# taqu/cpprcoder

Measured on AMD Instinct MI355X. Metric: MB/s encode+decode per GPU on 64 KiB blocks; ratio vs CPU ref, higher is better.
Workload: dtype u32

## Files before the change

### cpprcoder_amd/csrc/rcx_quad.hpp

```cpp
#pragma once

template <int CTRL>
__device__ __forceinline__ u32 rcx_dpp(u32 x)
{
    return (u32)__builtin_amdgcn_update_dpp(0, (int)x, CTRL, 0xF, 0xF, true);
}
__device__ __forceinline__ u32 rcx_oct_sum(u32 x)
{
    x += rcx_dpp<0xB1>(x);
    x += rcx_dpp<0x4E>(x);
    x += rcx_dpp<0x141>(x);
    return x;
}
__device__ __forceinline__ u32 rcx_oct_excl_scan(u32 x, u32 m1, u32 m2, u32 m4)
{
    u32 tot = x, pre = 0, o;
    o = rcx_dpp<0xB1>(tot);
    pre += o & m1;
    tot += o;
    o = rcx_dpp<0x4E>(tot);
    pre += o & m2;
    tot += o;
    o = rcx_dpp<0x141>(tot);
    pre += o & m4;
    return pre;
}

#define RCX_QUAD_BLOCKS 16
#define RCX_QUAD_GROUP_BYTES 4352
#define RCX_QUAD_RING_BYTES 144
#define RCX_QUAD_LDS_BYTES (4 * RCX_QUAD_GROUP_BYTES + RCX_QUAD_BLOCKS * RCX_QUAD_RING_BYTES)

typedef u32 RcxV4 __attribute__((ext_vector_type(4)));
typedef __attribute__((address_space(3))) RcxV4 RcxLdsV4;
typedef __attribute__((address_space(3))) u32 RcxLdsU32;
typedef RcxV4 RcxDivQv;
typedef RcxLdsV4 RcxLdsDivQ;

#define RCX_QUAD_DIVQ_DW 32

__device__ __forceinline__ u32 rcx_quad_sum(u32 x)
{
    x += rcx_dpp<0xB1>(x);
    x += rcx_dpp<0x4E>(x);
    return x;
}
__device__ __forceinline__ u32 rcx_umin(u32 a, u32 b) { return a < b ? a : b; }
__device__ __forceinline__ u32 rcx_umax(u32 a, u32 b) { return a > b ? a : b; }
__device__ __forceinline__ u32 rcx_quad_min(u32 x)
{
    x = rcx_umin(x, rcx_dpp<0xB1>(x));
    x = rcx_umin(x, rcx_dpp<0x4E>(x));
    return x;
}
__device__ __forceinline__ u32 rcx_quad_max(u32 x)
{
    x = rcx_umax(x, rcx_dpp<0xB1>(x));
    x = rcx_umax(x, rcx_dpp<0x4E>(x));
    return x;
}
__device__ __forceinline__ u32 rcx_quad_or(u32 x)
{
    x |= rcx_dpp<0xB1>(x);
    x |= rcx_dpp<0x4E>(x);
    return x;
}
__device__ __forceinline__ u32 rcx_quad_excl_scan(u32 x, u32 m1, u32 m2)
{
    u32 o = rcx_dpp<0xB1>(x);
    u32 pre = o & m1;
    const u32 tot = x + o;
    o = rcx_dpp<0x4E>(tot);
    pre += o & m2;
    return pre;
}

#if !defined(RCX_TOPUP_PIECES)
#define RCX_TOPUP_PIECES 1
#endif
struct QuadInput {
    u32 low, range;
    u32 bp8;
    u32 w0, w1;
    u32 n4;
    u32* ring;
    U4* skipped;
    u32 wr;
    u32 nfit;
    U4 pendA, pendB;
    const u8* origin;
    u32 last_off;
    u32 body8;

    __device__ __forceinline__ U4 load16(u32 off) const
    {
        return *reinterpret_cast<const U4*>(origin + (off < last_off ? off : last_off));
    }
    __device__ __forceinline__ void ring_put(const U4& piece, bool really)
    {
        const u32 slot = wr % RCX_RING_DW;
        *(really ? reinterpret_cast<U4*>(ring + slot) : skipped) = piece;
        ring[really && slot == 0 ? RCX_RING_DW : RCX_RING_DW + 1] = piece.x;
        wr += really ? 4u : 0u;
    }
    __device__ __forceinline__ void fetch_pair()
    {
        const u32* at = ring + ((bp8 >> 5) % RCX_RING_DW);
        w0 = at[0];
        w1 = at[1];
    }
    __device__ __forceinline__ u32 begin(const u8* s, const u8* stream_end, u32* block_ring, U4* scratch16)
    {
        skipped = scratch16;
        const u32 declared = (u32)s[0] | ((u32)s[1] << 8) | ((u32)s[2] << 16) | ((u32)s[3] << 24);
        low = ((u32)s[4] << 24) | ((u32)s[5] << 16) | ((u32)s[6] << 8) | (u32)s[7];
        range = 0x00FFFFFFu;
        ring = block_ring;
        const u8* body = s + 8;
        origin = body - ((uintptr_t)body & 15);
        last_off = (u32)(stream_end - 1 - origin) & ~15u;
        wr = 0;
        for (u32 r = 0; r < 6; ++r) ring_put(load16(16 * r), true);
        nfit = 0;
        pendA.x = pendA.y = pendA.z = pendA.w = 0;
        pendB = pendA;
        body8 = 8u * (u32)(body - origin);
        bp8 = body8;
        fetch_pair();
        n4 = rcx_bswap(rcx_funnel_shr(w1, w0, bp8));
        return declared;
    }
    __device__ __forceinline__ void idle(const u8* anywhere, u32* block_ring, U4* scratch16)
    {
        skipped = scratch16;
        low = 0;
        range = 0x01000000u;
        ring = block_ring;
        origin = anywhere - ((uintptr_t)anywhere & 15);
        last_off = 0;
        wr = 24;
        nfit = 0;
        pendA.x = pendA.y = pendA.z = pendA.w = 0;
        pendB = pendA;
        body8 = bp8 = 0;
        w0 = w1 = n4 = 0;
    }
    __device__ __forceinline__ void topup()
    {
        ring_put(pendA, nfit >= 1);
#if RCX_TOPUP_PIECES > 1
        ring_put(pendB, nfit >= 2);
#endif
        const u32 rd = bp8 >> 5;
        if (rcx_any(wr - rd < 14u)) {
            asm volatile("" ::: "memory");
            while (__any(wr - rd <= 20u)) ring_put(load16(4 * wr), wr - rd <= 20u);
        }
        const u32 room = (rd + RCX_RING_DW - wr) >> 2;
        nfit = room < (u32)RCX_TOPUP_PIECES ? room : (u32)RCX_TOPUP_PIECES;
        pendA = load16(4 * wr);
#if RCX_TOPUP_PIECES > 1
        pendB = load16(4 * wr + 16);
#endif
    }
    __device__ __forceinline__ u64 taken() const { return 8 + (u64)((bp8 - body8) >> 3); }
};

struct QuadSeat {
    u32 lane, wave;
    u32 quad, j;
    bool in_use;
    u64 blk;
    u8* lds;
    u8* mine;
    U4* leaves;
    U4* parked;
    u32* ring;
};
#define RCX_QUAD_SEAT(SEAT, WAVES, QUADS_USED, LDS_ALL, GEOM, NBLOCKS, N, BLOCK)                                       \
    QuadSeat SEAT;                                                                                                     \
    SEAT.lane = threadIdx.x & 63u;                                                                                     \
    SEAT.wave = __builtin_amdgcn_readfirstlane(threadIdx.x >> 6);                                                      \
    SEAT.lds = (LDS_ALL) + SEAT.wave * RCX_QUAD_LDS_BYTES;                                                             \
    SEAT.j = SEAT.lane & 3u, SEAT.quad = SEAT.lane >> 2;                                                               \
    SEAT.in_use = SEAT.quad < (QUADS_USED);                                                                            \
    SEAT.blk = ((u64)blockIdx.x * (WAVES) + SEAT.wave) * (QUADS_USED) + (SEAT.quad & ((QUADS_USED)-1u));               \
    RCX_ENTRY(GEOM, SEAT.blk, NBLOCKS, N, BLOCK);                                                                      \
    {                                                                                                                  \
                     \
        const u32 group = 2u * (SEAT.quad >> 3) + ((0x96u >> (SEAT.quad & 7u)) & 1u), quarter = (SEAT.quad & 7u) >> 1; \
        SEAT.mine = SEAT.lds + group * RCX_QUAD_GROUP_BYTES + quarter * 64;                                            \
        SEAT.leaves = reinterpret_cast<U4*>(SEAT.mine) + SEAT.j;                                                       \
        SEAT.parked = reinterpret_cast<U4*>(SEAT.mine + 16 * 256);                                                     \
        SEAT.ring = reinterpret_cast<u32*>(SEAT.lds + 4 * RCX_QUAD_GROUP_BYTES + SEAT.quad * RCX_QUAD_RING_BYTES);     \
    }

#define RCX_QUAD_FAIL(SEAT, GEOM, STATUS)                                                                              \
    {                                                                                                                  \
        if (SEAT.j == 0 && SEAT.in_use) rcx_flag(STATUS, RCX_ST_CORRUPT, rcx_id(GEOM, SEAT.blk));                      \
        live = false;                                                                                                  \
        len = 0;                                                                                                       \
    }
#define RCX_QUAD_MARK_REDO(SEAT, REDO, NBLOCKS, MARKED)                                                                \
    if (leader) (REDO)[SEAT.blk] = (MARKED) ? 1u : 0u;                                                                 \
    else if (SEAT.j == 0 && SEAT.in_use && SEAT.blk < (NBLOCKS)) (REDO)[SEAT.blk] = 0

#define RCX_QUAD_PARKED_FLUSH(I0, PARKED, LAST, ANY_ALIGN)                                                             \
    const u32 g = ((I0) >> 4) & 3u;                                                                                    \
    if (g == 0 && (I0) != 0 && leader) {                                                                               \
        u8* o4 = out + ((I0)-64);                                                                                      \
        const U4 p0 = (PARKED)[0], p1 = (PARKED)[1], p2 = (PARKED)[2];                                                 \
        rcx_store16<ANY_ALIGN>(o4, p0);                                                                                \
        rcx_store16<ANY_ALIGN>(o4 + 16, p1);                                                                           \
        rcx_store16<ANY_ALIGN>(o4 + 32, p2);                                                                           \
        rcx_store16<ANY_ALIGN>(o4 + 48, LAST);                                                                         \
    }
#define RCX_QUAD_PARKED_PUT(O, PARKED, LAST)                                                                           \
    if (g == 3) LAST = O;                                                                                              \
    else (PARKED)[g] = O
#define RCX_QUAD_PARKED_END(END, PARKED, LAST, ANY_ALIGN)                                                              \
    if (leader && (END) != 0) {                                                                                        \
        const u32 groups = (((END)-1) >> 4 & 3u) + 1;                                                                  \
        u8* o4 = out + (((END)-1) & ~63u);                                                                             \
        rcx_store16<ANY_ALIGN>(o4, (PARKED)[0]);                                                                       \
        if (groups > 1) rcx_store16<ANY_ALIGN>(o4 + 16, (PARKED)[1]);                                                  \
        if (groups > 2) rcx_store16<ANY_ALIGN>(o4 + 32, (PARKED)[2]);                                                  \
        if (groups > 3) rcx_store16<ANY_ALIGN>(o4 + 48, LAST);                                                         \
    }

#define RCX_QP1 "quad_perm:[1,0,3,2] row_mask:0xf bank_mask:0xf bound_ctrl:1\n\t"
#define RCX_QP2 "quad_perm:[2,3,0,1] row_mask:0xf bank_mask:0xf bound_ctrl:1\n\t"

#define RCX_QUAD_ROUND2_CUM(V, Q1, Q2, Q3, Q4)                                                                         \
    u32 lo_, rg_, nb_, hi_, y1_, y2_, y3_, y4_;                                                                       \
    asm volatile("v_sub_co_u32_e64 %[y1], %[c1], %[v], %[q1]\n\t"                                                     \
                 "v_sub_co_u32_e64 %[y2], %[c2], %[v], %[q2]\n\t"                                                     \
                 "v_sub_co_u32_e64 %[y3], %[c3], %[v], %[q3]\n\t"                                                     \
                 "v_sub_co_u32_e64 %[y4], %[c4], %[v], %[q4]\n\t"                                                     \
                 "v_subb_co_u32_e64 %[nb], %[c1], 4, 0, %[c1]\n\t"                                                    \
                 "v_min3_u32 %[lo], %[y1], %[y2], %[y3]\n\t"                                                          \
                 "v_subb_co_u32_e64 %[nb], %[c2], %[nb], 0, %[c2]\n\t"                                                \
                 "v_max3_u32 %[hi], %[y1], %[y2], %[y3]\n\t"                                                          \
                 "v_subb_co_u32_e64 %[nb], %[c3], %[nb], 0, %[c3]\n\t"                                                \
                 "v_min3_u32 %[lo], %[lo], %[y4], %[rem]\n\t"                                                         \
                 "v_subb_co_u32_e64 %[nb], %[c4], %[nb], 0, %[c4]\n\t"                                                \
                 "v_max_u32 %[hi], %[hi], %[y4]\n\t"                                                                  \
                 "v_min_u32_dpp %[lo], %[lo], %[lo] " RCX_QP1                                                         \
                 "v_add_u32_dpp %[nb], %[nb], %[nb] " RCX_QP1                                                         \
                 "v_max_u32_dpp %[hi], %[hi], %[hi] " RCX_QP1                                                         \
                 "v_min_u32_dpp %[lo], %[lo], %[lo] " RCX_QP2                                                         \
                 "v_add_u32_dpp %[nb], %[nb], %[nb] " RCX_QP2                                                         \
                 "v_max_u32_dpp %[hi], %[hi], %[hi] " RCX_QP2                                                         \
                 "v_sub_u32 %[rg], %[lo], %[hi]"                                                                      \
                 : [lo] "=&v"(lo_), [rg] "=&v"(rg_), [nb] "=&v"(nb_), [hi] "=&v"(hi_), [y1] "=&v"(y1_),               \
                   [y2] "=&v"(y2_), [y3] "=&v"(y3_), [y4] "=&v"(y4_), [c1] "=&s"(c1_), [c2] "=&s"(c2_),               \
                   [c3] "=&s"(c3_), [c4] "=&s"(c4_)                                                                   \
                 : [v] "v"(V), [q1] "v"(Q1), [q2] "v"(Q2), [q3] "v"(Q3), [q4] "v"(Q4),                                \
                   [rem] "v"(rem_));;

#define RCX_QUAD_16_SYMBOLS(SYMBOL, FINISH)                                                                            \
    SYMBOL(0, w0_, 0) SYMBOL(1, w0_, 0) SYMBOL(1, w0_, 8) SYMBOL(1, w0_, 16)                                           \
    SYMBOL(1, w0_, 24) SYMBOL(1, w1_, 0) SYMBOL(1, w1_, 8) SYMBOL(1, w1_, 16)                                          \
    SYMBOL(1, w1_, 24) SYMBOL(1, w2_, 0) SYMBOL(1, w2_, 8) SYMBOL(1, w2_, 16)                                          \
    SYMBOL(1, w2_, 24) SYMBOL(1, w3_, 0) SYMBOL(1, w3_, 8) SYMBOL(1, w3_, 16)                                          \
    FINISH(w3_, 24)

#define RCX_QUAD_TAIL(FROM, EACH, SYMBOL, FINISH, GATHER)                                                              \
    for (u32 i = (FROM); i < maxlen; ++i) {                                                                            \
        if ((i & 15u) == 0) in.topup();                                                                                \
        EACH                                                                                                           \
        if (i < len) {                                                                \
            u32 sym = 0;                                                                                               \
            SYMBOL(0, sym, 0);                                                                                         \
            FINISH(sym, 0);                                                                                            \
            sym = GATHER(sym);                                                                                         \
            if (leader) out[i] = (u8)sym;                                                                              \
        }                                                                                                              \
    }

#define RCX_QUAD_DEC_WAVES 4
template <int WAVES, class G = RcxBlocks>
__global__ __launch_bounds__(64 * WAVES) void rcx_dec_quad_k(const u8* __restrict__ comp, u64 comp_size, const u64* __restrict__ offsets,
                                                             u64 nblocks, u32 block, u64 n, u8* __restrict__ dst,
                                                             const u32* __restrict__ divq, u32* status,
                                                             u32* __restrict__ redo, u32 quads_used, const G g = G())
{
    __shared__ __attribute__((aligned(256))) u8 lds_all[WAVES * RCX_QUAD_LDS_BYTES];
    RCX_QUAD_SEAT(seat, WAVES, quads_used, lds_all, g, nblocks, n, block);

    {
        U4 v;
        v.x = v.y = v.z = v.w = ~0u;
#pragma unroll
        for (u32 q = 0; q < 17; ++q) seat.leaves[q * 16] = v;
    }
    u32 nU1 = 0u - (64u * seat.j + 16), nU2 = nU1 - 16, nU3 = nU1 - 32, nU4 = nU1 - 48;
    const u32 T0 = 4u * seat.j;
    const u32 m1 = (seat.j & 1u) ? ~0u : 0u, m2 = (seat.j & 2u) ? ~0u : 0u;

    QuadInput in;
    u64 stream_len = 0;
    if (live) {
        RCX_STREAM(g, seat.blk, offsets);
        if (!RCX_STREAM_OK(comp_size, 9)) {
            RCX_QUAD_FAIL(seat, g, status)
        } else {
            const u32 declared = in.begin(comp + s0, comp + s1, seat.ring, seat.parked + 3);
            if (declared != len) {
                RCX_QUAD_FAIL(seat, g, status)
            }
        }
    }
    if (!live) in.idle(comp, seat.ring, seat.parked + 3);

    const u32 maxlen = rcx_wave_max(len);
    u8* out = dst + at;
    u32 fast_end;
    {
        u32 mine = live ? (len & ~15u) : 0xFFFFFFF0u;
        if (!G::items && live && (reinterpret_cast<uintptr_t>(out) & 15u) != 0) mine = 0;
#pragma unroll
        for (int o = 32; o > 0; o >>= 1) {
            const u32 other = (u32)__shfl_xor((int)mine, o, 64);
            mine = mine < other ? mine : other;
        }
        fast_end = mine == 0xFFFFFFF0u ? 0u : mine;
    }
    const bool leader = live && seat.in_use && seat.j == 0;

    const u32 T0p3x4 = 4u * (T0 + 3);
    const u32 leaves_lds = (u32)reinterpret_cast<uintptr_t>(seat.leaves);
    const u32 ring_lds = (u32)reinterpret_cast<uintptr_t>(seat.ring);
#if defined(RCX_STAMP_DEC)
#define RCX_QUAD_STAMP(i) if (stamp_now_) stamp_t_[stamp_at_ + (i)] = __builtin_amdgcn_s_memtime();
#define RCX_QUAD_NO_STAMP                                                 \
    const bool stamp_now_ = false;                                                                         \
    const int stamp_at_ = 0;                                                                               \
    unsigned long long stamp_t_[4];
#else
#define RCX_QUAD_STAMP(i)
#define RCX_QUAD_NO_STAMP
#endif
    u32 p_hs_ = 0, p_sb4_ = 0, p_la_ = leaves_lds, p_own_ = 0;
#define RCX_QD_R_LO "v116"
#define RCX_QD_R_PAIR "{v[116:117]}"
    u64 R_ = 0;
#define RCX_QD_D "v[118:119]"
#define RCX_QD_D_L "v118"
#define RCX_QD_D_H "v119"
#define RCX_QD_YA "v[120:121]"
#define RCX_QD_YA_L "v120"
#define RCX_QD_YA_H "v121"
#define RCX_QD_YB "v[122:123]"
#define RCX_QD_YB_L "v122"
#define RCX_QD_YB_H "v123"
#define RCX_QD_YC "v[124:125]"
#define RCX_QD_YC_L "v124"
#define RCX_QD_YC_H "v125"
#define RCX_QD_YE "v[126:127]"
#define RCX_QD_YE_L "v126"
#define RCX_QD_YE_H "v127"
#define RCX_QD_PAIRS_CLOBBERED "v118", "v119", "v120", "v121", "v122", "v123", "v124", "v125", "v126", "v127"
#define RCX_QD_PREV_A_0 "s_nop 1\n\t"
#define RCX_QD_PREV_A_1 "v_lshl_add_u32 %[psym4], %[phs], 2, %[psb4]\n\t"                                           \
                        "v_bfi_b32 %[pad], 12, %[psym4], %[pla]\n\t"
#define RCX_QD_PREV_S_FIRST "v_and_b32 %[pword], %[psym4], %[pown]\n\t"                                             \
                            "v_lshrrev_b32 %[pword], 2, %[pword]\n\t"
#define RCX_QD_PREV_S_NEXT "v_and_b32 %[pye], %[psym4], %[pown]\n\t"                                                \
                           "v_lshl_or_b32 %[pword], %[pye], %[psh], %[pword]\n\t"
#define RCX_QP3 "quad_perm:[3,2,1,0] row_mask:0xf bank_mask:0xf bound_ctrl:1\n\t"
 \
#define RCX_QD_REM(PREV, PSHIFT, ...)                                                                      \
        asm volatile("v_min3_u32 %[rm], %[x1], %[x2], %[x3]\n\t"                                           \
                     "v_min3_u32 %[rm], %[rm], %[x4], %[low]\n\t"                                          \
                     "v_add_u32 %[u1], %[u1], %[h1]\n\t"                                                   \
                     "v_add_u32 %[u2], %[u2], %[h2]\n\t"                                                   \
                     "v_min_u32_dpp %[rm], %[rm], %[rm] " RCX_QP1                                          \
                     "v_add_u32 %[u3], %[u3], %[h3]\n\t"                                                   \
                     "v_add_u32 %[u4], %[u4], %[h4]\n\t"                                                   \
                     "v_min_u32_dpp " RCX_QD_R_LO ", %[rm], %[rm] " RCX_QP2  \
                     PREV                                                                                  \
                     : [u1] "+v"(nU1), [u2] "+v"(nU2), [u3] "+v"(nU3), [u4] "+v"(nU4), [rm] "=&v"(rem_),    \
                       [R] "+" RCX_QD_R_PAIR(R_) __VA_ARGS__                                                \
                     : [low] "v"(in.low), [x1] "v"(x1_), [x2] "v"(x2_),                                    \
                       [x3] "v"(x3_), [x4] "v"(x4_), [h1] "v"(h1_), [h2] "v"(h2_), [h3] "v"(h3_), [h4] "v"(h4_), \
                       [pown] "v"(p_own_), [psym4] "v"(psym4_), [psh] "n"((PSHIFT) > 2 ? (PSHIFT)-2 : 0))
#define RCX_QUAD_DEC_SYMBOL(MUL, INC, SH, HP, PWORD, PSHIFT)                                               \
    {                                                                                                      \
            \
        const u32 k8_ = rcx_clz(in.range) & 0x18u;                                                         \
        in.low = (u32)((((u64)in.low << 32) | in.n4) << k8_ >> 32);                                        \
                  \
        const u32 t_ = __umulhi((in.range << k8_) + (INC), (MUL)) >> (SH);                                 \
                                  \
        const u64 lowp_ = in.low;                                                                          \
        u32 node_, rem_, ro_, la_, pad_, pye_, psym4_;                                                     \
        u64 X1_, X2_, X3_, X4_, cz_, cy_;                                                                  \
        asm volatile("v_mad_i64_i32 %[X1], %[cz], %[n1], %[t], %[lp]\n\t"                                  \
                     "v_mad_i64_i32 %[X2], %[cz], %[n2], %[t], %[lp]\n\t"                                  \
                     "v_mad_i64_i32 %[X3], %[cz], %[n3], %[t], %[lp]\n\t"                                  \
                     "v_mad_i64_i32 %[X4], %[cz], %[n4], %[t], %[lp]"                                      \
                     : [X1] "=&v"(X1_), [X2] "=&v"(X2_), [X3] "=&v"(X3_), [X4] "=&v"(X4_), [cz] "=&s"(cz_)  \
                     : [n1] "v"(nU1), [n2] "v"(nU2), [n3] "v"(nU3), [n4] "v"(nU4), [t] "v"(t_), [lp] "v"(lowp_)); \
                                    \
        __builtin_amdgcn_sched_barrier(0);                                                                 \
        in.bp8 += k8_;                                                                                     \
        __builtin_amdgcn_sched_barrier(0);                                                                 \
        const u32 x1_ = (u32)X1_, x2_ = (u32)X2_, x3_ = (u32)X3_, x4_ = (u32)X4_;                          \
        const u32 h1_ = (u32)(X1_ >> 32), h2_ = (u32)(X2_ >> 32), h3_ = (u32)(X3_ >> 32), h4_ = (u32)(X4_ >> 32); \
        asm volatile("v_add3_u32 %[nd], %[h1], %[h2], %[h3]\n\t"                                           \
                     "v_add3_u32 %[nd], %[nd], %[h4], 4\n\t"  \
                     RCX_QD_PREV_A_##HP                                                                    \
                     : [nd] "=&v"(node_), [pad] "=&v"(pad_), [psym4] "=&v"(psym4_)                          \
                     : [h1] "v"(h1_), [h2] "v"(h2_), [h3] "v"(h3_), [h4] "v"(h4_),                         \
                       [phs] "v"(p_hs_), [psb4] "v"(p_sb4_), [pla] "v"(p_la_));                            \
        if (HP) (void)__hip_atomic_fetch_add(reinterpret_cast<RcxLdsU32*>(pad_), p_own_, __ATOMIC_RELAXED, __HIP_MEMORY_SCOPE_WAVEFRONT);  \
        asm volatile("v_add_u32_dpp %[nd], %[nd], %[nd] " RCX_QP1                                          \
                     "v_bfe_u32 %[ro], %[bp], 5, 5\n\t"                 \
                     "v_lshl_add_u32 %[ro], %[ro], 2, %[rb]"  \
                     : [nd] "+v"(node_), [ro] "=&v"(ro_)                                                    \
                     : [bp] "v"(in.bp8), [rb] "v"(ring_lds));                                              \
        {                                                                                                  \
            const RcxLdsU32* at_ = reinterpret_cast<const RcxLdsU32*>(ro_);  \
            in.w0 = at_[0];                                                                                \
            in.w1 = at_[1];                                                                                \
        }                                                                                                  \
        __builtin_amdgcn_sched_barrier(0);                                                                 \
        asm volatile("v_add_u32_dpp %[nd], %[nd], %[nd] " RCX_QP2                                          \
                     "v_lshl_add_u32 %[la], %[nd], 8, %[lvb]"  \
                     : [nd] "+v"(node_), [la] "=&v"(la_)                                                    \
                     : [lvb] "v"(leaves_lds));                                                             \
                                                              \
        RCX_QUAD_STAMP(0);                                                                                 \
        const RcxV4 l_ = *reinterpret_cast<const RcxLdsV4*>(la_);                                          \
        __builtin_amdgcn_sched_barrier(0);                                                                 \
        if (!(HP)) RCX_QD_REM("", 0);                                                                      \
        else if ((PSHIFT) == 0) RCX_QD_REM(RCX_QD_PREV_S_FIRST, 0, , [pword] "=&v"(PWORD));                \
        else RCX_QD_REM(RCX_QD_PREV_S_NEXT, PSHIFT, , [pye] "=&v"(pye_), [pword] "+v"(PWORD));             \
         \
         \
        u32 qe_, pre_, o2_, o3_;                                                                           \
        u32 lo_, rg_, hi_;                                                                                 \
        asm volatile("v_add3_u32 %[qe], %[lx], %[ly], %[lz]\n\t"                                           \
                     "v_add_u32 %[qe], %[qe], %[lw]\n\t"                                                   \
                     "v_alignbit_b32 %[n4], %[w1], %[w0], %[bp]\n\t"  \
                     "v_perm_b32 %[n4], %[n4], %[n4], %[swap]\n\t"  \
                     "v_and_b32_dpp %[pre], %[qe], %[m1] " RCX_QP1  \
                     "v_and_b32_dpp %[o2], %[qe], %[m2] " RCX_QP2                                          \
                     "v_and_b32_dpp %[o3], %[qe], %[m2] " RCX_QP3                                          \
                     "v_add3_u32 %[qe], %[pre], %[o2], %[o3]\n\t"                                         \
                     "v_mad_i64_i32 " RCX_QD_D ", %[cy], %[qe], %[t], %[R]\n\t"                             \
                     "v_mad_i64_i32 " RCX_QD_YA ", %[cy], %[lx], %[t], " RCX_QD_D "\n\t"                    \
                     "v_mad_i64_i32 " RCX_QD_YB ", %[cy], %[ly], %[t], " RCX_QD_YA "\n\t"                   \
                     "v_mad_i64_i32 " RCX_QD_YC ", %[cy], %[lz], %[t], " RCX_QD_YB "\n\t"                   \
                     "v_mad_i64_i32 " RCX_QD_YE ", %[cy], %[lw], %[t], " RCX_QD_YC "\n\t"                   \
                     "v_min3_u32 %[lo], " RCX_QD_D_L ", " RCX_QD_YA_L ", " RCX_QD_YB_L "\n\t"              \
                     "v_max3_u32 %[hi], " RCX_QD_YA_L ", " RCX_QD_YB_L ", " RCX_QD_YC_L "\n\t"             \
                     "v_min_u32 %[lo], %[lo], " RCX_QD_YC_L "\n\t"                                         \
                     "v_max_u32 %[hi], %[hi], " RCX_QD_YE_L "\n\t"                                         \
                     "v_add3_u32 %[hs], " RCX_QD_YA_H ", " RCX_QD_YB_H ", " RCX_QD_YC_H "\n\t"  \
                     "v_min_u32_dpp %[lo], %[lo], %[lo] " RCX_QP1                                          \
                     "v_max_u32_dpp %[hi], %[hi], %[hi] " RCX_QP1                                          \
                     "v_bfi_b32 %[own], " RCX_QD_D_H ", 0, " RCX_QD_YE_H "\n\t"  \
                     "v_min_u32_dpp %[lo], %[lo], %[lo] " RCX_QP2                                          \
                     "v_max_u32_dpp %[hi], %[hi], %[hi] " RCX_QP2                                          \
                     "v_sub_u32 %[rg], %[lo], %[hi]"                                                       \
                     : [n4] "=&v"(in.n4), [qe] "=&v"(qe_), [pre] "=&v"(pre_), [o2] "=&v"(o2_), [o3] "=&v"(o3_), \
                       [lo] "=&v"(lo_), [rg] "=&v"(rg_), [hs] "=&v"(p_hs_), [own] "=&v"(p_own_), [hi] "=&v"(hi_), \
                       [cy] "=&s"(cy_)                                                                      \
                     : [lx] "v"(l_.x), [ly] "v"(l_.y), [lz] "v"(l_.z), [lw] "v"(l_.w), [t] "v"(t_),        \
                       [R] "v"(R_), [m1] "v"(m1), [m2] "v"(m2),                                            \
                       [w0] "v"(in.w0), [w1] "v"(in.w1), [bp] "v"(in.bp8), [swap] "s"(0x00010203u)         \
                     : RCX_QD_PAIRS_CLOBBERED);                                                            \
                                  \
        __builtin_amdgcn_sched_barrier(0);                                                                 \
        p_sb4_ = (node_ << 6) + T0p3x4;                                                                    \
        __builtin_amdgcn_sched_barrier(0);                                                                 \
        asm volatile("" : : "v"(p_sb4_), "v"(qe_), "v"(pre_), "v"(o2_), "v"(o3_), "v"(hi_) : RCX_QD_PAIRS_CLOBBERED); \
        RCX_QUAD_STAMP(1);                                                                                 \
        in.low = lo_;                                                                            \
        in.range = rg_;                                                                          \
        p_la_ = la_;                                                                                       \
    }
#define RCX_QD_FINISH(BYTE, SHIFT, ...)                                                                    \
        asm volatile(RCX_QD_PREV_A_1                                                                       \
                     BYTE                                                                                  \
                     : [pad] "=&v"(pad_), [psym4] "=&v"(psym4_) __VA_ARGS__                                 \
                     : [pown] "v"(p_own_), [phs] "v"(p_hs_), [psb4] "v"(p_sb4_), [pla] "v"(p_la_),         \
                       [psh] "n"((SHIFT) > 2 ? (SHIFT)-2 : 0))
#define RCX_QUAD_DEC_FINISH(WORD, SHIFT)                                                                    \
    {                                                                                                      \
        u32 pad_, pye_, psym4_;                                                                            \
        if ((SHIFT) == 0) RCX_QD_FINISH(RCX_QD_PREV_S_FIRST, 0, , [pword] "=&v"(WORD));                    \
        else RCX_QD_FINISH(RCX_QD_PREV_S_NEXT, SHIFT, , [pye] "=&v"(pye_), [pword] "+v"(WORD));            \
        (void)__hip_atomic_fetch_add(reinterpret_cast<RcxLdsU32*>(pad_), p_own_, __ATOMIC_RELAXED, __HIP_MEMORY_SCOPE_WAVEFRONT);  \
    }

#if defined(RCX_QUAD_DIV_SMEM)
    const u32* dq_ = divq;
#else
    u32 vz_;
    asm volatile("v_mov_b32 %0, 0" : "=v"(vz_));
    const u32* dq_ = divq + vz_;
#endif
#define RCX_QUAD_DIVQ_LOAD(G, Q)                                                                             \
    {                                                                                                      \
        __builtin_amdgcn_sched_barrier(0);                                                                 \
        dm##Q = reinterpret_cast<const U4*>(dq_ + (G) * RCX_QUAD_DIVQ_DW)[Q];                              \
        di##Q = reinterpret_cast<const U4*>(dq_ + (G) * RCX_QUAD_DIVQ_DW + 16)[Q];                         \
    }
#define RCX_QUAD_U4_AT(V, C) ((C) == 0 ? (V).x : (C) == 1 ? (V).y : (C) == 2 ? (V).z : (V).w)
    {
        U4 o_last;
        o_last.x = o_last.y = o_last.z = o_last.w = 0;
#if defined(RCX_STAMP_DEC)
        unsigned long long stamp_sum_[4] = {0, 0, 0, 0};
#endif
        U4 dm0, dm1, dm2, dm3, di0, di1, di2, di3;
        RCX_QUAD_DIVQ_LOAD(0u, 0) RCX_QUAD_DIVQ_LOAD(0u, 1) RCX_QUAD_DIVQ_LOAD(0u, 2) RCX_QUAD_DIVQ_LOAD(0u, 3)
        asm volatile("" ::"v"(dm0.x), "v"(di0.x), "v"(dm1.x), "v"(di1.x), "v"(dm2.x), "v"(di2.x), "v"(dm3.x), "v"(di3.x));
#if defined(RCX_STAMP_DEC)
#define RCX_QUAD_STEP(S, Q, HP, PW)                                                                           \
    {                                                                                                        \
        const bool stamp_now_ = (S) == 8 || (S) == 9;                                                        \
        const int stamp_at_ = (S) == 8 ? 0 : 2;                                                              \
        RCX_QUAD_DEC_SYMBOL(RCX_QUAD_U4_AT(dm##Q, (S) & 3), RCX_QUAD_U4_AT(di##Q, (S) & 3), sh_, HP, PW,     \
                            (8 * (((S) + 3) & 3)));                                                          \
    }
#else
#define RCX_QUAD_STEP(S, Q, HP, PW)                                                                           \
    RCX_QUAD_DEC_SYMBOL(RCX_QUAD_U4_AT(dm##Q, (S) & 3), RCX_QUAD_U4_AT(di##Q, (S) & 3), sh_, HP, PW, (8 * (((S) + 3) & 3)));
#endif
#define RCX_QUAD_GROUP(GN, O)                                                                                 \
    {                                                                                                        \
        u32 w0_ = 0, w1_ = 0, w2_ = 0, w3_ = 0;                                                              \
        RCX_QUAD_STEP(0, 0, 0, w0_) RCX_QUAD_STEP(1, 0, 1, w0_) RCX_QUAD_STEP(2, 0, 1, w0_) RCX_QUAD_STEP(3, 0, 1, w0_) \
        RCX_QUAD_DIVQ_LOAD(GN, 0)                                                                            \
        RCX_QUAD_STEP(4, 1, 1, w0_) RCX_QUAD_STEP(5, 1, 1, w1_) RCX_QUAD_STEP(6, 1, 1, w1_) RCX_QUAD_STEP(7, 1, 1, w1_) \
        RCX_QUAD_DIVQ_LOAD(GN, 1)                                                                            \
        RCX_QUAD_STEP(8, 2, 1, w1_) RCX_QUAD_STEP(9, 2, 1, w2_) RCX_QUAD_STEP(10, 2, 1, w2_) RCX_QUAD_STEP(11, 2, 1, w2_) \
        RCX_QUAD_DIVQ_LOAD(GN, 2)                                                                            \
        RCX_QUAD_STEP(12, 3, 1, w2_) RCX_QUAD_STEP(13, 3, 1, w3_) RCX_QUAD_STEP(14, 3, 1, w3_) RCX_QUAD_STEP(15, 3, 1, w3_) \
        RCX_QUAD_DIVQ_LOAD(GN, 3)                                                                            \
        RCX_QUAD_DEC_FINISH(w3_, 24)                                                                         \
        (O).x = rcx_quad_or(w0_);                                                                            \
        (O).y = rcx_quad_or(w1_);                                                                            \
        (O).z = rcx_quad_or(w2_);                                                                            \
        (O).w = rcx_quad_or(w3_);                                                                            \
    }
        u32 i0 = 0;
#if !defined(RCX_STAMP_DEC)
        {
            U4 o_p0 = o_last, o_p1 = o_last, o_p2 = o_last;
            for (; i0 + 64 <= fast_end; i0 += 64) {
                in.topup();
                if (i0 != 0 && leader) {
                    u8* o4 = out + (i0 - 64);
                    rcx_store16<G::items>(o4, o_p0);
                    rcx_store16<G::items>(o4 + 16, o_p1);
                    rcx_store16<G::items>(o4 + 32, o_p2);
                    rcx_store16<G::items>(o4 + 48, o_last);
                }
                const u32 sh_ = 31u - (u32)__builtin_clz(256u + i0);
                const u32 gn_ = (i0 >> 4) + 1u;
                RCX_QUAD_GROUP(gn_, o_p0)
                in.topup();
                RCX_QUAD_GROUP(gn_ + 1u, o_p1)
                in.topup();
                RCX_QUAD_GROUP(gn_ + 2u, o_p2)
                in.topup();
                RCX_QUAD_GROUP(gn_ + 3u, o_last)
            }
            if (i0 != 0) seat.parked[0] = o_p0, seat.parked[1] = o_p1, seat.parked[2] = o_p2;
        }
#endif
        for (; i0 < fast_end; i0 += 16) {
            in.topup();
            RCX_QUAD_PARKED_FLUSH(i0, seat.parked, o_last, G::items)
            const u32 sh_ = 31u - (u32)__builtin_clz(256u + i0);
            const u32 gn_ = (i0 >> 4) + 1u;
#if defined(RCX_STAMP_DEC)
            unsigned long long stamp_t_[4] = {0, 0, 0, 0};
#endif
            U4 o;
            RCX_QUAD_GROUP(gn_, o)
#if defined(RCX_STAMP_DEC)
            stamp_sum_[0] += stamp_t_[1] - stamp_t_[0];
            stamp_sum_[1] += stamp_t_[2] - stamp_t_[1];
            stamp_sum_[2] += stamp_t_[3] - stamp_t_[2];
            stamp_sum_[3] += 1;
#endif
            RCX_QUAD_PARKED_PUT(o, seat.parked, o_last);
        }
#undef RCX_QUAD_GROUP
#undef RCX_QUAD_STEP
#if defined(RCX_STAMP_DEC)
        if (blockIdx.x == 7 && threadIdx.x == 0)
            for (int i_ = 0; i_ < 4; ++i_) rcx_dec_stamp_out[i_] = stamp_sum_[i_];
#endif
        RCX_QUAD_PARKED_END(fast_end, seat.parked, o_last, G::items)
    }
    {
        u32 mul_n_, inc_n_;
#define RCX_QUAD_DIVQ_ENTRY(I)                                                                              \
    {                                                                                                      \
        const u32* e_ = divq + ((I) >> 4) * RCX_QUAD_DIVQ_DW + ((I) & 15u);                                 \
        mul_n_ = e_[0];                                                                                    \
        inc_n_ = e_[16];                                                                                   \
    }
        RCX_QUAD_DIVQ_ENTRY(fast_end);
#define RCX_QUAD_TAIL_EACH                                                                                  \
    const u32 mul_ = mul_n_, inc_ = inc_n_, sh_ = 31u - (u32)__builtin_clz(256u + i);                      \
    RCX_QUAD_DIVQ_ENTRY(i + 1u);                                                                           \
    RCX_QUAD_NO_STAMP
#define RCX_QUAD_TAIL_SYMBOL(HP, WORD, SHIFT) RCX_QUAD_DEC_SYMBOL(mul_, inc_, sh_, HP, WORD, SHIFT)
        RCX_QUAD_TAIL(fast_end, RCX_QUAD_TAIL_EACH, RCX_QUAD_TAIL_SYMBOL, RCX_QUAD_DEC_FINISH, rcx_quad_or)
#undef RCX_QUAD_TAIL_EACH
#undef RCX_QUAD_TAIL_SYMBOL
    }
#undef RCX_QUAD_DEC_SYMBOL
#undef RCX_QUAD_DEC_FINISH
#undef RCX_QD_PREV_A_0
#undef RCX_QD_PREV_A_1
#undef RCX_QD_PREV_S_FIRST
#undef RCX_QD_PREV_S_NEXT
#undef RCX_QD_REM
#undef RCX_QD_FINISH
#undef RCX_QD_R_LO
#undef RCX_QD_R_PAIR
#undef RCX_QD_D
#undef RCX_QD_D_L
#undef RCX_QD_D_H
#undef RCX_QD_YA
#undef RCX_QD_YA_L
#undef RCX_QD_YA_H
#undef RCX_QD_YB
#undef RCX_QD_YB_L
#undef RCX_QD_YB_H
#undef RCX_QD_YC
#undef RCX_QD_YC_L
#undef RCX_QD_YC_H
#undef RCX_QD_YE
#undef RCX_QD_YE_L
#undef RCX_QD_YE_H
#undef RCX_QD_PAIRS_CLOBBERED
#undef RCX_QP3
#undef RCX_QUAD_DIVQ_LOAD
#undef RCX_QUAD_DIVQ_ENTRY
#undef RCX_QUAD_U4_AT
    const bool marked = live && rcx_quad_or(seat.j == 3 && 0u - nU4 != 256u + len ? 1u : 0u) != 0;
    if (leader && !marked && in.taken() > stream_len) rcx_flag(status, RCX_ST_CORRUPT, rcx_id(g, seat.blk));
    RCX_QUAD_MARK_REDO(seat, redo, nblocks, marked);
}
```

Before: 84250.

## Overlap quad-group merge with next group's first symbol decode; scalarize loop bounds

Result: no change. 84150 (-0.1%).

```diff
diff --git a/cpprcoder_amd/csrc/rcx_quad.hpp b/cpprcoder_amd/csrc/rcx_quad.hpp
--- a/cpprcoder_amd/csrc/rcx_quad.hpp
+++ b/cpprcoder_amd/csrc/rcx_quad.hpp
@@ -152,7 +152,7 @@
         ring_put(pendB, nfit >= 2);
 #endif
         const u32 rd = bp8 >> 5;
-        if (rcx_any(wr - rd < 14u)) {
+        if (__builtin_expect(rcx_any(wr - rd < 14u), 0)) {
             asm volatile("" ::: "memory");
             while (__any(wr - rd <= 20u)) ring_put(load16(4 * wr), wr - rd <= 20u);
         }
@@ -313,7 +313,7 @@
     }
     if (!live) in.idle(comp, seat.ring, seat.parked + 3);
 
-    const u32 maxlen = rcx_wave_max(len);
+    const u32 maxlen = __builtin_amdgcn_readfirstlane(rcx_wave_max(len));
     u8* out = dst + at;
     u32 fast_end;
     {
@@ -325,6 +325,7 @@
             mine = mine < other ? mine : other;
         }
         fast_end = mine == 0xFFFFFFF0u ? 0u : mine;
+        fast_end = __builtin_amdgcn_readfirstlane(fast_end);
     }
     const bool leader = live && seat.in_use && seat.j == 0;
 
@@ -520,10 +521,17 @@
         RCX_QUAD_DIVQ_LOAD(0u, 0) RCX_QUAD_DIVQ_LOAD(0u, 1) RCX_QUAD_DIVQ_LOAD(0u, 2) RCX_QUAD_DIVQ_LOAD(0u, 3)
         asm volatile("" ::"v"(dm0.x), "v"(di0.x), "v"(dm1.x), "v"(di1.x), "v"(dm2.x), "v"(di2.x), "v"(dm3.x), "v"(di3.x));
 #if defined(RCX_STAMP_DEC)
+#if defined(RCX_STAMP_DEC_BOUNDARY)
+#define RCX_QUAD_STAMPED(S) ((S) == 15 || (S) == 0)
+#define RCX_QUAD_STAMP_SLOT(S) ((S) == 15 ? 0 : 2)
+#else
+#define RCX_QUAD_STAMPED(S) ((S) == 8 || (S) == 9)
+#define RCX_QUAD_STAMP_SLOT(S) ((S) == 8 ? 0 : 2)
+#endif
 #define RCX_QUAD_STEP(S, Q, HP, PW)                                                                           \
     {                                                                                                        \
-        const bool stamp_now_ = (S) == 8 || (S) == 9;                                                        \
-        const int stamp_at_ = (S) == 8 ? 0 : 2;                                                              \
+        const bool stamp_now_ = RCX_QUAD_STAMPED(S);                                                         \
+        const int stamp_at_ = RCX_QUAD_STAMP_SLOT(S);                                                        \
         RCX_QUAD_DEC_SYMBOL(RCX_QUAD_U4_AT(dm##Q, (S) & 3), RCX_QUAD_U4_AT(di##Q, (S) & 3), sh_, HP, PW,     \
                             (8 * (((S) + 3) & 3)));                                                          \
     }
@@ -531,25 +539,36 @@
 #define RCX_QUAD_STEP(S, Q, HP, PW)                                                                           \
     RCX_QUAD_DEC_SYMBOL(RCX_QUAD_U4_AT(dm##Q, (S) & 3), RCX_QUAD_U4_AT(di##Q, (S) & 3), sh_, HP, PW, (8 * (((S) + 3) & 3)));
 #endif
+#define RCX_QUAD_GROUP_OPEN(GN, W0, W1, W2, W3, HP0, PW0, AFTER0)                                             \
+    {                                                                                                        \
+        RCX_QUAD_STEP(0, 0, HP0, PW0) AFTER0                                                                 \
+        RCX_QUAD_STEP(1, 0, 1, W0) RCX_QUAD_STEP(2, 0, 1, W0) RCX_QUAD_STEP(3, 0, 1, W0)                     \
+        RCX_QUAD_DIVQ_LOAD(GN, 0)                                                                            \
+        RCX_QUAD_STEP(4, 1, 1, W0) RCX_QUAD_STEP(5, 1, 1, W1) RCX_QUAD_STEP(6, 1, 1, W1) RCX_QUAD_STEP(7, 1, 1, W1) \
+        RCX_QUAD_DIVQ_LOAD(GN, 1)                                                                            \
+        RCX_QUAD_STEP(8, 2, 1, W1) RCX_QUAD_STEP(9, 2, 1, W2) RCX_QUAD_STEP(10, 2, 1, W2) RCX_QUAD_STEP(11, 2, 1, W2) \
+        RCX_QUAD_DIVQ_LOAD(GN, 2)                                                                            \
+        RCX_QUAD_STEP(12, 3, 1, W2) RCX_QUAD_STEP(13, 3, 1, W3) RCX_QUAD_STEP(14, 3, 1, W3) RCX_QUAD_STEP(15, 3, 1, W3) \
+        RCX_QUAD_DIVQ_LOAD(GN, 3)                                                                            \
+    }
+#define RCX_QUAD_GROUP_MERGE(O)                                                                               \
+    (O).x = rcx_quad_or((O).x), (O).y = rcx_quad_or((O).y), (O).z = rcx_quad_or((O).z), (O).w = rcx_quad_or((O).w);
 #define RCX_QUAD_GROUP(GN, O)                                                                                 \
-    {                                                                                                        \
-        u32 w0_ = 0, w1_ = 0, w2_ = 0, w3_ = 0;                                                              \
-        RCX_QUAD_STEP(0, 0, 0, w0_) RCX_QUAD_STEP(1, 0, 1, w0_) RCX_QUAD_STEP(2, 0, 1, w0_) RCX_QUAD_STEP(3, 0, 1, w0_) \
-        RCX_QUAD_DIVQ_LOAD(GN, 0)                                                                            \
-        RCX_QUAD_STEP(4, 1, 1, w0_) RCX_QUAD_STEP(5, 1, 1, w1_) RCX_QUAD_STEP(6, 1, 1, w1_) RCX_QUAD_STEP(7, 1, 1, w1_) \
-        RCX_QUAD_DIVQ_LOAD(GN, 1)                                                                            \
-        RCX_QUAD_STEP(8, 2, 1, w1_) RCX_QUAD_STEP(9, 2, 1, w2_) RCX_QUAD_STEP(10, 2, 1, w2_) RCX_QUAD_STEP(11, 2, 1, w2_) \
-        RCX_QUAD_DIVQ_LOAD(GN, 2)                                                                            \
-        RCX_QUAD_STEP(12, 3, 1, w2_) RCX_QUAD_STEP(13, 3, 1, w3_) RCX_QUAD_STEP(14, 3, 1, w3_) RCX_QUAD_STEP(15, 3, 1, w3_) \
-        RCX_QUAD_DIVQ_LOAD(GN, 3)                                                                            \
-        RCX_QUAD_DEC_FINISH(w3_, 24)                                                                         \
-        (O).x = rcx_quad_or(w0_);                                                                            \
-        (O).y = rcx_quad_or(w1_);                                                                            \
-        (O).z = rcx_quad_or(w2_);                                                                            \
-        (O).w = rcx_quad_or(w3_);                                                                            \
-    }
+    RCX_QUAD_GROUP_OPEN(GN, (O).x, (O).y, (O).z, (O).w, 0, (O).x, RCX_QUAD_STAMP_BOUNDARY(0))                \
+    RCX_QUAD_DEC_FINISH((O).w, 24)                                                                           \
+    RCX_QUAD_GROUP_MERGE(O)
+#if defined(RCX_STAMP_DEC_BOUNDARY)
+        unsigned long long stamp_t_[4] = {0, 0, 0, 0};
+#define RCX_QUAD_STAMP_BOUNDARY(INSIDE)                                                                       \
+    if (stamp_t_[1] != 0) {                                                                                  \
+        stamp_sum_[(INSIDE) ? 0 : 1] += stamp_t_[2] - stamp_t_[1];                                           \
+        stamp_sum_[(INSIDE) ? 3 : 2] += 1;                                                                   \
+    }
+#else
+#define RCX_QUAD_STAMP_BOUNDARY(INSIDE)
+#endif
         u32 i0 = 0;
-#if !defined(RCX_STAMP_DEC)
+#if !defined(RCX_STAMP_DEC) || defined(RCX_STAMP_DEC_BOUNDARY)
         {
             U4 o_p0 = o_last, o_p1 = o_last, o_p2 = o_last;
             for (; i0 + 64 <= fast_end; i0 += 64) {
@@ -563,13 +582,15 @@
                 }
                 const u32 sh_ = 31u - (u32)__builtin_clz(256u + i0);
                 const u32 gn_ = (i0 >> 4) + 1u;
-                RCX_QUAD_GROUP(gn_, o_p0)
+                RCX_QUAD_GROUP_OPEN(gn_, o_p0.x, o_p0.y, o_p0.z, o_p0.w, 0, o_p0.x, RCX_QUAD_STAMP_BOUNDARY(0))
                 in.topup();
-                RCX_QUAD_GROUP(gn_ + 1u, o_p1)
+                RCX_QUAD_GROUP_OPEN(gn_ + 1u, o_p1.x, o_p1.y, o_p1.z, o_p1.w, 1, o_p0.w, RCX_QUAD_STAMP_BOUNDARY(1) RCX_QUAD_GROUP_MERGE(o_p0))
                 in.topup();
-                RCX_QUAD_GROUP(gn_ + 2u, o_p2)
+                RCX_QUAD_GROUP_OPEN(gn_ + 2u, o_p2.x, o_p2.y, o_p2.z, o_p2.w, 1, o_p1.w, RCX_QUAD_STAMP_BOUNDARY(1) RCX_QUAD_GROUP_MERGE(o_p1))
                 in.topup();
-                RCX_QUAD_GROUP(gn_ + 3u, o_last)
+                RCX_QUAD_GROUP_OPEN(gn_ + 3u, o_last.x, o_last.y, o_last.z, o_last.w, 1, o_p2.w, RCX_QUAD_STAMP_BOUNDARY(1) RCX_QUAD_GROUP_MERGE(o_p2))
+                RCX_QUAD_DEC_FINISH(o_last.w, 24)
+                RCX_QUAD_GROUP_MERGE(o_last)
             }
             if (i0 != 0) seat.parked[0] = o_p0, seat.parked[1] = o_p1, seat.parked[2] = o_p2;
         }
@@ -579,12 +600,12 @@
             RCX_QUAD_PARKED_FLUSH(i0, seat.parked, o_last, G::items)
             const u32 sh_ = 31u - (u32)__builtin_clz(256u + i0);
             const u32 gn_ = (i0 >> 4) + 1u;
-#if defined(RCX_STAMP_DEC)
+#if defined(RCX_STAMP_DEC) && !defined(RCX_STAMP_DEC_BOUNDARY)
             unsigned long long stamp_t_[4] = {0, 0, 0, 0};
 #endif
             U4 o;
             RCX_QUAD_GROUP(gn_, o)
-#if defined(RCX_STAMP_DEC)
+#if defined(RCX_STAMP_DEC) && !defined(RCX_STAMP_DEC_BOUNDARY)
             stamp_sum_[0] += stamp_t_[1] - stamp_t_[0];
             stamp_sum_[1] += stamp_t_[2] - stamp_t_[1];
             stamp_sum_[2] += stamp_t_[3] - stamp_t_[2];
@@ -592,6 +613,9 @@
 #endif
             RCX_QUAD_PARKED_PUT(o, seat.parked, o_last);
         }
+#undef RCX_QUAD_GROUP_OPEN
+#undef RCX_QUAD_GROUP_MERGE
+#undef RCX_QUAD_STAMP_BOUNDARY
 #undef RCX_QUAD_GROUP
 #undef RCX_QUAD_STEP
 #if defined(RCX_STAMP_DEC)
```
